# articulatory/articulatory

Measured on AMD Instinct MI355X. Metric: audio samples/sec (16 kHz) EMA->wav HiFi-CAR, batch 64, higher is better.
Workload: dtype fp32; 1 GPU; configs[2]: HiFi-CAR (e2w_hifigan_car.yaml generator) 13-dim pitch+EMA -> 16 kHz, batch 64/GPU, 10 s clips, 80 sequential chunks of 25 frames; batch_per_gpu=64, frames=2000, chunk_frames=25, weights=synthetic seed 1234 (articulatory_amd.utils.synth), parallelism=utterance-sharded x1, arithmetic=exact fp32 products (v_mfma_f32_32x32x2_f32), fp32 accumulate, gather=none

## Files before the change

__graft_entry__.py:

```python

import os
import subprocess
import sys

REPO = os.path.dirname(os.path.abspath(__file__))
if REPO not in sys.path:
    sys.path.insert(0, REPO)


def build() -> None:
    csrc = os.path.join(REPO, "articulatory_amd", "csrc")
    subprocess.run(["make", "-C", csrc, f"-j{max(1, min(11, os.cpu_count() or 1))}"], check=True)
    import articulatory_amd
    from articulatory_amd import _native

    lib = _native.load_library()
    for sym in _native.SYMBOLS:
        getattr(lib, sym)
    print("built", _native.LIB_PATH, lib.hificar_version().decode())


def smoke() -> None:
    import numpy as np
    import torch

    from articulatory_amd.models import HiFiGANGenerator
    from articulatory_amd.utils.synth import synth_features, synth_state_dict
# ... 47 lines not shown
```

articulatory_amd/csrc/hificar.hip:

```cpp
#include "hificar_kernels.hip.h"
#include "hificar_launch.h"
#include "hificar_backward.hip.h"
#include "hificar_disc_kernels.hip.h"

#include "../../include/hificar.h"

#include <algorithm>
#include <queue>
#include <cmath>
#include <cstdarg>
#include <cstdio>
#include <cstring>
#include <functional>
#include <map>
#include <string>
#include <vector>

using namespace hificar;

static thread_local char g_err[1024] = "";

static int fail(int code, const char* fmt, ...) {
    va_list ap;
    va_start(ap, fmt);
// ... 44 lines not shown
struct hificar_handle {
    hificar_config cfg;
    int arch = 0;
    std::vector<GBlockLayers> gb;
    int c_last = 0;
    bool finalized = false;
    int precision = HIFICAR_PREC_F32;
    bool profile_detail = false;
    bool use_pair = true;
    bool use_lpt = true;
    double mi1_penalty = 1.05;
    int pick_throughput = 0;
    bool xcd_order = true;
    bool pair_small = true;
    int ksplit = 1;
    int cf = 0;
    int cin_pad = 0;
    int hop = 1;
    int num_cus = 256;
    std::map<std::string, std::vector<int64_t>> expected;
    std::map<std::string, HostTensor> tensors;
    ConvLayer input_conv;
    std::vector<ConvLayer> ups;
    std::vector<ConvLayer> convs1;
    std::vector<ConvLayer> convs2;
    float* d_out_w = nullptr;
    float out_bias = 0.f;
    float* d_out_bias = nullptr;
    void* train = nullptr;
    void (*train_free)(hificar_handle*) = nullptr;
// ... 62 lines not shown
    hipStream_t prof_stream = nullptr;
};

static FILE* g_launch_log = nullptr;
static void read_env_switches(hificar_handle* h) {
    if (const char* e = getenv("HIFICAR_PROFILE_DETAIL")) h->profile_detail = atoi(e) != 0;
    if (const char* e = getenv("HIFICAR_LAUNCH_LOG")) {
        if (!g_launch_log && *e) g_launch_log = fopen(e, "a");
        if (g_launch_log) h->profile_detail = true;
    }
    if (const char* e = getenv("HIFICAR_KSPLIT")) h->ksplit = atoi(e);
    if (const char* e = getenv("HIFICAR_PAIR")) h->use_pair = atoi(e) != 0;
    if (const char* e = getenv("HIFICAR_PAIR_SMALL")) h->pair_small = atoi(e) != 0;
    if (const char* e = getenv("HIFICAR_AR_DUAL_MIN")) h->ar_dual_min = atoi(e);
    if (const char* e = getenv("HIFICAR_AR_DUAL_MAX")) h->ar_dual_max = atoi(e);
}

struct ProfScope {
    hificar_handle* h;
    hipStream_t s;
    hipEvent_t e0 = nullptr, e1 = nullptr;
    std::string name;
    double flops, bytes;
    ProfScope(hificar_handle* h_, hipStream_t s_, const std::string& n, double f, double b) : h(h_), s(s_), name(n), flops(f), bytes(b) {
        if (g_launch_log) {
            fprintf(g_launch_log, "%s\t%.0f\t%.0f\n", n.c_str(), f, b);
            fflush(g_launch_log);
        }
        if (!h->profiling) return;
        (void)hipEventCreate(&e0);
// ... 376 lines not shown
    if (!L.transposed && L.cin_pad == L.cin && (L.cin == 32 || L.cin == 64) && L.cout == L.cin) {
        if ((rc = pack_w16(h, L, W, L.cin_pad, &L.d_w16c)) != HIFICAR_OK) return rc;
        if ((rc = pack_w32(h, L, W, L.cin_pad, &L.d_w32c)) != HIFICAR_OK) return rc;
    }
    return HIFICAR_OK;
}

hipError_t hificar::conv_launch(const ConvShape& s, const void* params, dim3 grid, size_t lds_bytes, hipStream_t stream) {
    bool handled = false;
    hipError_t e = hipSuccess;
#define HIFICAR_TRY_SET(n)                                                      \
    if (!handled) e = conv_inst_launch_##n(s, params, grid, lds_bytes, stream, &handled); \
    if (handled) return e;
    HIFICAR_TRY_SET(0) HIFICAR_TRY_SET(1) HIFICAR_TRY_SET(2) HIFICAR_TRY_SET(3) HIFICAR_TRY_SET(4)
    HIFICAR_TRY_SET(5) HIFICAR_TRY_SET(6) HIFICAR_TRY_SET(7) HIFICAR_TRY_SET(8) HIFICAR_TRY_SET(9)
#undef HIFICAR_TRY_SET
    return hipErrorInvalidValue;
}

hipError_t hificar::conv_set_lds_attributes() {
    hipError_t e = hipSuccess;
#define HIFICAR_ATTR_SET(n) \
    if (e == hipSuccess) e = conv_inst_attrs_##n();
    HIFICAR_ATTR_SET(0) HIFICAR_ATTR_SET(1) HIFICAR_ATTR_SET(2) HIFICAR_ATTR_SET(3) HIFICAR_ATTR_SET(4)
    HIFICAR_ATTR_SET(5) HIFICAR_ATTR_SET(6) HIFICAR_ATTR_SET(7) HIFICAR_ATTR_SET(8) HIFICAR_ATTR_SET(9)
#undef HIFICAR_ATTR_SET
    return e;
}

static int engine_setup(hificar_handle* h) {
    {
        void* z = nullptr;
        HIP_TRY(hipMalloc(&z, 256));
        h->allocs.push_back(z);
        HIP_TRY(hipMemset(z, 0, 256));
        h->d_zeros = static_cast<char*>(z);
    }
    HIP_TRY(conv_set_lds_attributes());
    if (h->arenas.empty()) {
        int rca = arena_add(h, 0);
// ... 347 lines not shown
    float mask_slope = 0.f;
    long long x_seq_bytes = 0;
    int x_row_bytes = 0;
    int x_rows = 0;
    int x_up = 0;
    float x_slope = -1.f;
    const float* x_more[3] = {nullptr, nullptr, nullptr};
    int x_n = 1;
};

struct ConvRep {
    int n = 1;
    long long zs_x = 0, zs_w = 0, zs_y = 0, zs_b = 0;
};

static int launch_conv(hificar_handle* h, const ConvLayer* const* layers, int nbr, int nseq, int rows, const ConvIO* io,
                              float slope_out, const Ragged& rg, hipStream_t stream, const ConvRep& zr = ConvRep()) {
    const ConvLayer& L0 = *layers[0];
    const bool f32 = h->precision == HIFICAR_PREC_F32;
    int halo_all = 0;
    for (int b = 0; b < nbr; ++b) halo_all = std::max(halo_all, layers[b]->off_max - layers[b]->off_min);
    TileCfg tc = {1, 4, 1, 1, 1};
    double best = 1e300;
    int best_ti = 11;
    const int nsteps_min = [&] {
        int m = 1 << 30;
        for (int b = 0; b < nbr; ++b) m = std::min(m, layers[b]->ntaps * (L0.chunk16 / 16));
        return m;
    }();
    std::string pick_key;
    pick_key.reserve(160);
    pick_key += f32 ? 'f' : 'c';
    pick_key += h->train ? 't' : 'i';
    if (h->shared_chip) pick_key += 's';
    for (int b = 0; b < nbr; ++b) {
        pick_key += '|';
        pick_key += layers[b]->name;
    }
    pick_key += '|' + std::to_string(nseq) + 'x' + std::to_string(rows) + 'z' + std::to_string(zr.n);
    const auto cached_pick = h->tile_picks.find(pick_key);
    if (cached_pick != h->tile_picks.end()) tc = kTileCfgs[cached_pick->second];
    else
    for (int ti = 0; ti < kNumTileCfgs; ++ti) {
        const TileCfg& t = kTileCfgs[ti];
        const int TM = t.WM * t.MI * 32;
        const int chunk = L0.chunk16, RB = chunk * 4;
        if (t.NB == 2 && (f32 || L0.chunk16 == 16)) continue;
        const size_t obuf = (f32 && t.KS == 1) ? 0 : out_buf_bytes(t);
        if (2 * round_up_sz((size_t)(TM + halo_all) * RB, 1024) + obuf > 160 * 1024) continue;
        if (t.NB == 2) {
            bool ok = L0.n_blocks32 >= 2;
            for (int b = 0; b < nbr; ++b) ok = ok && (layers[b]->n_phase == 1 || layers[b]->nb32_per_phase % 2 == 0);
            if (!ok) continue;
        }
        if (t.KS == 4 && (h->ksplit == 0 || nsteps_min < 2)) continue;
        if (t.KS == 1 && h->ksplit == 2 && nsteps_min >= 2) continue;
        const long long tiles_per_branch = (long long)nseq * ((rows + TM - 1) / TM) * ((L0.n_blocks32 + t.WN * t.NB - 1) / (t.WN * t.NB));
        const long long total = tiles_per_branch * nbr * zr.n;
        const int G = (int)std::min<long long>(total, h->num_cus);
        const int nchunks = L0.cin_pad / chunk;
        double total_cost = 0.0, heaviest = 0.0, lightest = 1e300, cb[3] = {0.0, 0.0, 0.0};
        for (int b = 0; b < nbr; ++b) {
            const double slab = f32 ? 8 * 64.0 : 3 * 32 / 0.75;
            double c = (double)layers[b]->ntaps * (L0.cin_pad / 16) * slab * t.MI * t.NB + 2500.0 + 400.0 * nchunks;
            if (t.KS == 4) {
                const int steps = layers[b]->ntaps * (chunk / 16);
                c = (double)((steps + 3) / 4) * nchunks * slab * t.MI + 4000.0 + 600.0 * nchunks;
            }
            total_cost += c * tiles_per_branch * zr.n;
            heaviest = std::max(heaviest, c);
            lightest = std::min(lightest, c);
            cb[b] = c;
        }
        double worst = std::max(heaviest, total_cost / G);
        if (h->use_lpt && !h->shared_chip && total > G && total <= 4096) {
            std::sort(cb, cb + nbr, [](double x, double y) { return x > y; });
            std::priority_queue<double, std::vector<double>, std::greater<double>> load;
            for (int w = 0; w < G; ++w) load.push(0.0);
            worst = 0.0;
            for (int b = 0; b < nbr; ++b)
                for (long long i = 0; i < tiles_per_branch * zr.n; ++i) {
                    const double v = load.top() + cb[b];
                    load.pop();
                    load.push(v);
                    worst = std::max(worst, v);
                }
        } else if (total % G != 0) {
            worst = std::max(worst, total_cost / G + 0.5 * lightest);
        }
        if (h->pick_throughput > 0 && total >= h->pick_throughput) worst = total_cost / h->num_cus;
        if (t.NB == 2) worst *= f32 ? (t.MI == 4 ? 0.95 : t.MI == 2 ? 0.975 : 1.02) : (t.MI == 2 ? 0.93 : 1.10);
        else if (t.MI < 4) worst *= f32 ? (t.MI == 2 ? 1.02 : h->mi1_penalty) : (t.MI == 2 ? 1.10 : 1.25);
        if (t.KS == 4) worst *= 1.05;
        if (worst < best * 0.98) {
            best = worst;
            tc = t;
            best_ti = ti;
        }
    }
    if (cached_pick == h->tile_picks.end()) {
        if (h->tile_picks.size() > 20000) h->tile_picks.clear();
        h->tile_picks.emplace(pick_key, best_ti);
    }
    const int TM = tc.WM * tc.MI * 32;
    const int chunk_sel = L0.chunk16, RB = chunk_sel * 4;
    const int nc16 = chunk_sel / 16;
    MultiConvParams mp;
    memset(&mp, 0, sizeof(mp));
    double flops = 0.0, bytes = 0.0;
    for (int b = 0; b < nbr; ++b) {
        const ConvLayer& Lb = *layers[b];
        if (Lb.n_blocks32 != L0.n_blocks32 || Lb.chunk16 != L0.chunk16 || Lb.cin_pad != L0.cin_pad)
            return fail(HIFICAR_E_INVALID, "internal: branch shape mismatch");
        fill_params(mp.p[b], Lb, rows, TM, io[b].res, io[b].y, rg);
        mp.p[b].xs = io[b].xs;
        mp.p[b].ys = io[b].ys;
        if (io[b].x_slope >= 0.f) {
            if (!f32) return fail(HIFICAR_E_INVALID, "internal: pre-activation input rows of %s outside the exact-fp32 layer-by-layer launches", Lb.name.c_str());
// ... 33 lines not shown
    mp.buf_bytes = (int)buf_bytes;
    mp.trace = nullptr;
    mp.zrep = zr.n;
    mp.zs_x = zr.zs_x;
    mp.zs_w = zr.zs_w;
    mp.zs_y = zr.zs_y;
    mp.zs_b = zr.zs_b;
    dim3 grid((unsigned)std::min(mp.total_tiles, h->num_cus), 1, 1);
    {
        double wbytes = 0.0;
        for (int b = 0; b < nbr; ++b) wbytes += 4.0 * layers[b]->cin_pad * layers[b]->cout_total * layers[b]->ntaps * zr.n;
        const double abytes = 4.0 * nseq * rows * L0.cin_pad * nbr * zr.n;
        mp.xcd_order = (h->xcd_order && mp.total_tiles <= h->num_cus && mp.total_tiles >= 16 && wbytes > 2.0 * abytes) ? 1 : 0;
    }
    mp.stage_cached = mp.ngroups > 2 ? 1 : 0;
    if (mp.total_tiles <= h->num_cus && nbr == 1 && zr.n == 1 && mp.ngroups >= 2 && mp.nseq_tiles >= 8 && !h->shared_chip) {
        const double wbytes1 = 4.0 * L0.cin_pad * L0.cout_total * L0.ntaps;
        if (wbytes1 > 6.0e6) {
            const int R = mp.nseq_tiles, Gc = mp.ngroups;
            int bpr = 1, bpg = 8;
            double bcost = 1e300;
            for (int pr = 1; pr <= 8; pr *= 2) {
                const int pg = 8 / pr;
                if (pr > R || pg > Gc) continue;
                const double c = (double)((R + pr - 1) / pr) + (double)((Gc + pg - 1) / pg);
                if (c < bcost) bcost = c, bpr = pr, bpg = pg;
            }
            std::vector<std::vector<int>> per_xcd(8);
            size_t maxblock = 0;
            for (int x = 0; x < 8; ++x) {
// ... 19 lines not shown
    if (!mp.sched_start && h->use_lpt && mp.total_tiles > (int)grid.x) {
        std::vector<double> costs((size_t)mp.total_tiles);
        const int tpb = mp.ngroups * mp.nseq_tiles;
        std::string key = f32 ? "f" : "c";
        for (int b = 0; b < nbr; ++b) {
            key += "|" + layers[b]->name;
            for (int i = 0; i < tpb * zr.n; ++i) costs[(size_t)b * tpb * zr.n + i] = layers[b]->ntaps + 1.0;
        }
        if (zr.n > 1) key += "z" + std::to_string(zr.n);
        key += "|" + std::to_string(nseq) + "x" + std::to_string((rows + TM - 1) / TM) + "t" + std::to_string(TM) + "w" + std::to_string(tc.WN) +
               "k" + std::to_string(tc.KS) + (tc.NB == 2 ? "b" : "");
        int rc2 = get_schedule(h, key, costs, (int)grid.x, stream, &mp.sched_start, &mp.sched_tiles);
        if (rc2 != HIFICAR_OK) return rc2;
    }
    char kname[96];
    if (dout) snprintf(kname, sizeof(kname), "conv_f32do_kernel<%d,%d,%d,%d>", tc.MI, tc.WM, tc.WN, nc16);
    else if (tc.KS == 4) snprintf(kname, sizeof(kname), "%s<%d,%d>", f32 ? "conv_sk_f32_kernel" : "conv_sk_bf16x3_kernel", tc.MI, nc16);
    else if (tc.NB == 2) snprintf(kname, sizeof(kname), "conv_bf16x3nb_kernel<%d,%d,%d,%d>", tc.MI, tc.WM, tc.WN, nc16);
    else snprintf(kname, sizeof(kname), "conv_bf16x3_kernel<%d,%d,%d,%d>", tc.MI, tc.WM, tc.WN, nc16);
    if (h->profile_detail) {
        const size_t n = strlen(kname);
        snprintf(kname + n, sizeof(kname) - n, "|%s x%d", L0.name.c_str(), nbr);
    }
    ProfScope prof(h, stream, kname, flops, bytes);
    const ConvShape shape = {dout ? kConvF32do : tc.KS == 4 ? (f32 ? kConvSkF32 : kConvSkBf16x3) : tc.NB == 2 ? kConvBf16x3nb : kConvBf16x3,
                             tc.MI, tc.WM, tc.WN, nc16};
    const hipError_t e = conv_launch(shape, &mp, grid, lds, stream);
    if (e != hipSuccess) return fail(HIFICAR_E_HIP, "conv launch (%s, %s) failed: %s", L0.name.c_str(), kname, hipGetErrorString(e));
    return HIFICAR_OK;
}

struct PairIOB {
    const float* xf;
    const char* xs;
    const float* res;
    float* y;
    char* ys;
};

static bool pair_small_tiles(const hificar_handle* h, int C, int k2, int nseq, int rows) {
    if (!h->pair_small || h->ksplit == 0 || C != 32 || h->precision != HIFICAR_PREC_F32 || nseq <= 0 || (long long)nseq * rows < 8000) return false;
    const int tmo = 4 * 4 * 32 - (k2 - 1);
// ... 249 lines not shown
            h->tap_scratch = static_cast<float*>(p);
            h->tap_scratch_elems = need;
        }
        if (cfg.use_ar && (rc = emit_tap(h, "ar_feats", ws.xin, f32 ? h->cin_pad : -h->cin_pad, h->cf, cfg.ar_output, B, 1, f32 ? 0 : 1, stream, T)) != HIFICAR_OK)
            return rc;
    }
    const size_t tap_se = tapping ? stage_elems(h, B, T) : 0;
    const int nbk = cfg.n_blocks;
    int order[kMaxBlk];
    for (int j = 0; j < kMaxBlk; ++j) order[j] = j;
    std::sort(order, order + nbk, [&](int a, int b) { return cfg.resblock_kernel_sizes[a] > cfg.resblock_kernel_sizes[b]; });
    int max_d = 0;
    for (int j = 0; j < nbk; ++j) max_d = std::max(max_d, cfg.n_dilations[j]);
    int rows_of_launch = 0;
    const bool add_convs = cfg.use_additional_convs != 0;
    auto conv_n = [&](const ConvLayer* const* lay, int n, const ConvIO* io) -> int {
        for (int q0 = 0; q0 < n; q0 += 3) {
            const int r = launch_conv(h, lay + q0, std::min(3, n - q0), B, rows_of_launch, io + q0, cfg.lrelu_slope, rg, stream);
            if (r != HIFICAR_OK) return r;
        }
        return HIFICAR_OK;
    };

    const float* fin[kMaxBlk] = {ws.x[0], ws.x[1], ws.x[2], ws.x[3]};
    {
        char* xin_s = tp ? reinterpret_cast<char*>(tp->xin) : reinterpret_cast<char*>(ws.xin);
        char* h0_s = tp ? tp->h0_s : reinterpret_cast<char*>(ws.h0);
        char* xt_s[kMaxBlk] = {reinterpret_cast<char*>(ws.xt[0]), reinterpret_cast<char*>(ws.xt[1]), reinterpret_cast<char*>(ws.xt[2]),
                               reinterpret_cast<char*>(ws.xt[3])};
        {
            const ConvLayer* lay[1] = {&h->input_conv};
            float* y_tap = tap_wanted(h, "input_conv") ? h->tap_scratch + kMaxBlk * tap_se : nullptr;
            const ConvIO io[1] = {{xin_s, nullptr, y_tap, h0_s}};
            if ((rc = launch_conv(h, lay, 1, B, T, io, cfg.lrelu_slope, rg, stream)) != HIFICAR_OK) return rc;
            if (y_tap && (rc = emit_tap(h, "input_conv", y_tap, stage_pad(cfg, 0), 0, cfg.channels, B, T, 0, stream)) != HIFICAR_OK) return rc;
        }
        for (int i = 0; i < cfg.n_stages; ++i) {
            const char* up_in = h0_s;
            const bool fold_mrf = i > 0 && f32 && !tp;
            if (i > 0 && !fold_mrf) {
                MrfSplitParams mq;
                memset(&mq, 0, sizeof(mq));
                mq.x0 = fin[0];
                mq.x1 = nbk > 1 ? fin[1] : nullptr;
                mq.x2 = nbk > 2 ? fin[2] : nullptr;
                mq.x3 = nbk > 3 ? fin[3] : nullptr;
                mq.out = fin[0] == ws.xt[0] ? ws.x_s[0] : xt_s[0];
                if (tp) mq.out = tp->upin_s[i];
                mq.nin = nbk;
                mq.C = stage_pad(cfg, i);
                mq.rows = (long long)B * rows;
                mq.slope = cfg.lrelu_slope;
                mq.f32 = f32 ? 1 : 0;
                const long long units = mq.rows * (mq.C / 8);
// ... 2 lines not shown
                    ProfScope prof(h, stream, "mrf_split_kernel", 0.0, 4.0 * mq.rows * mq.C * (nbk + 1));
                    hipLaunchKernelGGL(mrf_split_kernel, dim3(blocks), dim3(256), 0, stream, mq);
                }
                HIP_TRY(hipGetLastError());
                up_in = mq.out;
            }
            bool all_pairs = !tap_convs1 && !tp && add_convs;
            for (int j = 0; j < nbk && all_pairs; ++j)
                for (int d = 0; d < cfg.n_dilations[j]; ++d) {
                    const int ci = conv_index(h, i, j, d);
                    all_pairs = all_pairs && pair_eligible(h, h->convs1[ci], h->convs2[ci], B, rows * cfg.upsample_scales[i]);
                }
            {
                const ConvLayer* lay[1] = {&h->ups[i]};
                ConvIO io[1] = {{up_in, nullptr, ws.u, all_pairs ? nullptr : (tp ? tp->u_s[i] : ws.u_s)}};
                if (fold_mrf) {
                    io[0].xs = reinterpret_cast<const char*>(fin[0]);
                    io[0].x_slope = cfg.lrelu_slope;
                    io[0].x_n = nbk;
                    for (int j = 1; j < nbk; ++j) io[0].x_more[j - 1] = fin[j];
                }
                if ((rc = launch_conv(h, lay, 1, B, rows, io, cfg.lrelu_slope, rg, stream)) != HIFICAR_OK) return rc;
            }
            rows *= cfg.upsample_scales[i];
            const int Cs = stage_channels(cfg, i + 1), Cp = stage_pad(cfg, i + 1);
            if (tapping && (rc = emit_tap(h, "upsamples." + std::to_string(i), ws.u, Cp, 0, Cs, B, rows, 0, stream)) != HIFICAR_OK) return rc;
            auto tap_block = [&](int j, int d, const float* xcur) -> int {
                if (!tapping) return HIFICAR_OK;
                const std::string base = "blocks." + std::to_string(i * nbk + j);
                int r = emit_tap(h, base + ".x." + std::to_string(d), xcur, Cp, 0, Cs, B, rows, 0, stream);
                if (r == HIFICAR_OK && d + 1 == cfg.n_dilations[j]) r = emit_tap(h, base, xcur, Cp, 0, Cs, B, rows, 0, stream);
// ... 19 lines not shown
                    }
                    for (int q0 = 0; q0 < n; q0 += 3)
                        if ((rc = launch_pair(h, l1 + q0, l2 + q0, std::min(3, n - q0), B, rows, iop + q0, cfg.lrelu_slope, rg, stream)) != HIFICAR_OK) return rc;
                    for (int j = 0; j < nbk; ++j)
                        if (d < cfg.n_dilations[j] && (rc = tap_block(j, d, cur_f[j])) != HIFICAR_OK) return rc;
                }
                for (int j = 0; j < nbk; ++j) fin[j] = cur_f[j];
                continue;
            }
            float* xres[kMaxBlk] = {ws.x[0], ws.x[1], ws.x[2], ws.x[3]};
            if (tp && i + 1 == cfg.n_stages)
                for (int j = 0; j < nbk; ++j) xres[j] = tp->fin[j];
            for (int j = 0; j < nbk; ++j) fin[j] = xres[j];
            const char* u_act = tp ? tp->u_s[i] : ws.u_s;
            const char* cur_s[kMaxBlk] = {u_act, u_act, u_act, u_act};
            for (int d = 0; d < max_d; ++d) {
                const ConvLayer* l1[kMaxBlk];
                const ConvLayer* l2[kMaxBlk];
                ConvIO io1[kMaxBlk], io2[kMaxBlk];
                PairIOB iop[kMaxBlk];
                int jn[kMaxBlk];
                char* pair_out[kMaxBlk];
                char* lbl_out[kMaxBlk];
                int n = 0;
                bool fuse = add_convs;
                for (int oj = 0; oj < nbk; ++oj) {
                    const int j = order[oj];
                    if (d >= cfg.n_dilations[j]) continue;
                    const int ci = conv_index(h, i, j, d);
                    l1[n] = &h->convs1[ci];
// ... 6 lines not shown
                    if (tp) {
                        mid = tp->xt_s[i][j][d];
                        lbl_out[n] = tp->x_s[i][j][d];
                    }
                    io1[n] = {cur_s[j], nullptr, tap_convs1 ? h->tap_scratch + (size_t)n * tap_se : nullptr, mid};
                    io2[n] = {mid, d == 0 ? ws.u : xres[j], xres[j], last ? nullptr : lbl_out[n]};
                    if (!add_convs) {
                        char* nxt = tp ? tp->x_s[i][j][d] : pair_out[n];
                        io1[n] = {cur_s[j], d == 0 ? ws.u : xres[j], xres[j], last ? nullptr : nxt};
                        lbl_out[n] = nxt;
                    }
                    iop[n] = {nullptr, cur_s[j], d == 0 ? ws.u : xres[j], xres[j], last ? nullptr : pair_out[n]};
                    jn[n] = j;
                    ++n;
                }
                if (fuse) {
                    for (int q0 = 0; q0 < n; q0 += 3)
                        if ((rc = launch_pair(h, l1 + q0, l2 + q0, std::min(3, n - q0), B, rows, iop + q0, cfg.lrelu_slope, rg, stream)) != HIFICAR_OK) return rc;
                } else if (!add_convs) {
                    rows_of_launch = rows;
                    if ((rc = conv_n(l1, n, io1)) != HIFICAR_OK) return rc;
                } else {
                    rows_of_launch = rows;
                    if ((rc = conv_n(l1, n, io1)) != HIFICAR_OK) return rc;
                    if (tap_convs1)
                        for (int q = 0; q < n; ++q)
                            if ((rc = emit_tap(h, "blocks." + std::to_string(i * nbk + jn[q]) + ".convs1." + std::to_string(d), io1[q].y, Cp, 0, Cs,
                                               B, rows, 0, stream)) != HIFICAR_OK)
                                return rc;
                    if ((rc = conv_n(l2, n, io2)) != HIFICAR_OK) return rc;
                }
                for (int q = 0; q < n; ++q)
                    if ((rc = tap_block(jn[q], d, xres[jn[q]])) != HIFICAR_OK) return rc;
                for (int q = 0; q < n; ++q) cur_s[jn[q]] = fuse ? pair_out[q] : lbl_out[q];
            }
        }
    }
    if (cfg.use_ph_loss && cond.ph_out) {
        PhHeadParams pq;
        memset(&pq, 0, sizeof(pq));
        pq.x0 = fin[0];
        pq.x1 = nbk > 1 ? fin[1] : nullptr;
        pq.x2 = nbk > 2 ? fin[2] : nullptr;
        pq.x3 = nbk > 3 ? fin[3] : nullptr;
        pq.nin = nbk;
        pq.w = h->d_phfc_w;
// ... 287 lines not shown
```

articulatory_amd/csrc/hificar_conv.hip.h:

```cpp
#pragma once
#include <hip/hip_runtime.h>
#include <stdint.h>
#include <type_traits>

namespace hificar {

typedef float f32x2 __attribute__((ext_vector_type(2)));
typedef float f32x4 __attribute__((ext_vector_type(4)));
typedef unsigned u32x4_t __attribute__((ext_vector_type(4)));
typedef float f32x16 __attribute__((ext_vector_type(16)));
typedef __bf16 bf16x4 __attribute__((ext_vector_type(4)));
typedef __bf16 bf16x8 __attribute__((ext_vector_type(8)));

constexpr int kMaxPhase = 8;
constexpr int kMaxTaps = 16;

struct ConvParams {
    const bf16x8* w16;
    const float* bias;
    const float* res;
    const float* mask_src;
    float mask_slope;
    float* y;
    const float* xf;
// ... 51 lines not shown
    ConvParams p[3];
    int n_branches;
    int nseq_tiles;
    int ngroups;
    int total_tiles;
    int buf_bytes;
    const int* sched_start;
    const int* sched_tiles;
    int zrep;
    long long zs_x, zs_w, zs_y, zs_b;
    unsigned long long* trace;
    int xcd_order;
    int stage_cached;
};


#ifdef HIFICAR_TRACE
__device__ unsigned long long g_trace_realtime[2][1024];
__device__ unsigned long long g_trace_rt_slots[4][64];
#define HIFICAR_STAMP(slot)                                                                            \
    do {                                                                                               \
        if (mp.trace && lane == 0 && (wave == 0 || wave == kFirstLoader) && (slot) < 64)               \
            mp.trace[((size_t)blockIdx.x * 2 + (wave ? 1 : 0)) * 64 + (slot)] = __builtin_amdgcn_s_memtime(); \
        if (mp.trace && lane == 0 && wave == 0 && ((slot) == 0 || (slot) == 63) && blockIdx.x < 1024)  \
            g_trace_realtime[(slot) == 63][blockIdx.x] = __builtin_amdgcn_s_memrealtime();             \
        if (mp.trace && lane == 0 && wave == 0 && (slot) < 64 && blockIdx.x < 4)                       \
            g_trace_rt_slots[blockIdx.x][(slot)] = __builtin_amdgcn_s_memrealtime();                   \
    } while (0)
#else
#define HIFICAR_STAMP(slot) do { } while (0)
// ... 9 lines not shown
        constexpr int lo = NMEM * I / NMFMA, hi = NMEM * (I + 1) / NMFMA;
        constexpr int ds = (hi < NDS ? hi : NDS) - (lo < NDS ? lo : NDS);
        constexpr int vm = (hi - lo) - ds;
        __builtin_amdgcn_sched_group_barrier(0x008, 1, 0);
        if constexpr (ds > 0) __builtin_amdgcn_sched_group_barrier(0x100, ds, 0);
        if constexpr (vm > 0) __builtin_amdgcn_sched_group_barrier(0x020, vm, 0);
        pin_slab_slot<I + 1, NDS, NVMEM, NMFMA>();
    }
}
template <int NDS, int NVMEM, int NMFMA>
__device__ __forceinline__ void pin_slab_step() {
    pin_slab_slot<0, NDS, NVMEM, NMFMA>();
}
__device__ __forceinline__ void lds_barrier() { asm volatile("s_waitcnt lgkmcnt(0)\n\ts_barrier" ::: "memory"); }

template <int MI, int WM, int WN, int NC16, bool F32, int KS = 1, int NB = 1, bool DOUT = false>
__device__ __forceinline__ void conv_ws_body(const MultiConvParams& mp) {
    static_assert(!DOUT || (F32 && KS == 1 && NB == 1), "direct output: exact fp32, dense form, one channel block per wave");
    static_assert(NB == 1 || (NB == 2 && KS == 1), "one or two channel blocks per MFMA wave");
    static_assert(KS == 1 || (KS == 4 && WM == 1 && WN == 1), "split-K: four waves share one 32-channel block");
    static_assert(KS == 4 || WM * WN == 4 || WM * WN == 8, "4 or 8 MFMA waves per workgroup");
    constexpr int NW = KS == 4 ? 4 : WM * WN;
    constexpr bool kPrimeOnce = DOUT;
    constexpr bool kRowMajorAcc = DOUT;
    constexpr int NTHR = (NW + 4) * 64;
    constexpr int kFirstLoader = NW;
    (void)kFirstLoader;
    static_assert(NC16 == 1 || NC16 == 2 || NC16 == 4, "chunk of 16, 32 or 64 channels");
    constexpr int TM = WM * MI * 32;
    constexpr int CH = NC16 * 16;
    constexpr int RB = CH * 4;
    constexpr int SPR = CH / 4;
    constexpr int LOG_SPR = NC16 == 4 ? 4 : NC16 == 2 ? 3 : 2;
// ... 30 lines not shown
        const unsigned tps = (unsigned)mp.p[0].tiles_per_seq;
        const unsigned seq = m / tps;
        T.seq = (int)seq;
        T.t0 = (int)((m - seq * tps) * (unsigned)TM);
        return T;
    };

    constexpr int TN = WN * NB * 32;
    constexpr int OP = TN + 4;
    int sched_lo = 0, sched_hi = 0;
    if (mp.sched_start) scalar_load_2i32(mp.sched_start + blockIdx.x, sched_lo, sched_hi);
    const int my_rounds = mp.sched_start ? sched_hi - sched_lo
                                         : (mp.total_tiles - (int)blockIdx.x + (int)gridDim.x - 1) / (int)gridDim.x;
    auto tile_of = [&](int it) {
        int i = it;
        if ((blockIdx.x & 1) && my_rounds >= 3 && it >= my_rounds - 2) i = it == my_rounds - 1 ? my_rounds - 2 : my_rounds - 1;
        if (mp.sched_start) return scalar_load_i32(mp.sched_tiles + sched_lo + i);
        if (mp.xcd_order) {
            const int x = (int)blockIdx.x & 7, l = (int)blockIdx.x >> 3;
            const int base = mp.total_tiles >> 3, rem = mp.total_tiles & 7;
            return x * base + min(x, rem) + l;
        }
        return (int)blockIdx.x + (my_rounds - 1 - i) * (int)gridDim.x;
    };
    auto nxt = [&](int i) {
        if (is_ragged(mp.p[0]))
            while (i < my_rounds) {
                const Tile T = decode(tile_of(i));
                if (T.t0 < seq_rows(mp.p[T.b], T.seq)) break;
                ++i;
            }
// ... 410 lines not shown
                    for (int m0 = 0; m0 < MI; m0 += G2) {
                        float rs[G2][16], mk[G2][16];
                        if constexpr (kRes || kMask) {
#pragma unroll
                            for (int mm = 0; mm < G2; ++mm)
#pragma unroll
                                for (int r = 0; r < 16; ++r) fetch1(m0 + mm, r, rs[mm], mk[mm]);
                        }
#pragma unroll
                        for (int mm = 0; mm < G2; ++mm)
#pragma unroll
                            for (int r = 0; r < 16; ++r) finish(m0 + mm, r, rs[mm], mk[mm]);
                    }
                }
            };
            constexpr std::true_type Y{};
            constexpr std::false_type N{};
            if (has_mask) {
                pass(Y, Y, Y, Y);
                return;
            }
            if (has_res) {
                if (has_y && has_ys) pass(Y, N, Y, Y);
                else if (has_y) pass(Y, N, Y, N);
                else pass(Y, N, N, Y);
            } else {
                if (has_y && has_ys) pass(N, N, Y, Y);
                else if (has_y) pass(N, N, Y, N);
                else pass(N, N, N, Y);
            }
// ... 232 lines not shown
    }
    lds_barrier();
    HIFICAR_STAMP(62);
    if constexpr (!DOUT) {
        if (last >= 0) write_out(decode(tile_of(last)), tid, NTHR);
    }
    HIFICAR_STAMP(63);
}

template <int MI, int WM, int WN, int NC16>
__global__ __launch_bounds__((WM * WN + 4) * 64) void conv_f32do_kernel(const MultiConvParams mp) {
    conv_ws_body<MI, WM, WN, NC16, true, 1, 1, true>(mp);
}

template <int MI, int WM, int WN, int NC16>
__global__ __launch_bounds__((WM * WN + 4) * 64) void conv_bf16x3_kernel(const MultiConvParams mp) {
    conv_ws_body<MI, WM, WN, NC16, false>(mp);
}

template <int MI, int WM, int WN, int NC16>
__global__ __launch_bounds__((WM * WN + 4) * 64) void conv_bf16x3nb_kernel(const MultiConvParams mp) {
    conv_ws_body<MI, WM, WN, NC16, false, 1, 2>(mp);
}

template <int MI, int NC16>
__global__ __launch_bounds__(512) void conv_sk_bf16x3_kernel(const MultiConvParams mp) {
    conv_ws_body<MI, 1, 1, NC16, false, 4>(mp);
}

template <int MI, int NC16>
// ... 476 lines not shown
```

articulatory_amd/csrc/hificar_conv_inst.hip:

```cpp
#include "hificar_conv.hip.h"
#include "hificar_launch.h"

#ifndef HIFICAR_INST_SET
#error "compile with -DHIFICAR_INST_SET=0..9"
#endif

namespace hificar {

#define HIFICAR_TILES9(X, nc) X(4, 1, 4, nc) X(4, 2, 2, nc) X(4, 4, 1, nc) X(2, 1, 4, nc) X(2, 2, 2, nc) X(2, 4, 1, nc) X(1, 1, 4, nc) X(1, 2, 2, nc) X(1, 4, 1, nc)

#if HIFICAR_INST_SET == 0
#define FAMILY kConvF32do
#define KERNEL conv_f32do_kernel
#define PARAMS MultiConvParams
#define SHAPES(X) HIFICAR_TILES9(X, 1)
#elif HIFICAR_INST_SET == 1
#define FAMILY kConvF32do
#define KERNEL conv_f32do_kernel
#define PARAMS MultiConvParams
#define SHAPES(X) HIFICAR_TILES9(X, 2)
#elif HIFICAR_INST_SET == 2
#define FAMILY kConvF32do
#define KERNEL conv_f32do_kernel
#define PARAMS MultiConvParams
// ... 17 lines not shown
#define FAMILY kConvBf16x3nb
#define KERNEL conv_bf16x3nb_kernel
#define PARAMS MultiConvParams
#define SHAPES(X) X(2, 2, 2, 2) X(2, 4, 1, 2) X(2, 1, 4, 2) X(2, 2, 2, 4) X(2, 4, 1, 4) X(2, 1, 4, 4)
#elif HIFICAR_INST_SET == 7 || HIFICAR_INST_SET == 8
#if HIFICAR_INST_SET == 7
#define FAMILY kConvSkF32
#define KERNEL_PTR(mi, wm, wn, nc) (conv_sk_f32_kernel<mi, nc>)
#else
#define FAMILY kConvSkBf16x3
#define KERNEL_PTR(mi, wm, wn, nc) (conv_sk_bf16x3_kernel<mi, nc>)
#endif
#define THREADS(wm, wn) 512
#define PARAMS MultiConvParams
#define SHAPES(X) X(1, 1, 1, 1) X(2, 1, 1, 1) X(4, 1, 1, 1) X(1, 1, 1, 2) X(2, 1, 1, 2) X(4, 1, 1, 2) X(1, 1, 1, 4) X(2, 1, 1, 4) X(4, 1, 1, 4)
#elif HIFICAR_INST_SET == 9
#define PARAMS PairParams
#define THREADS(wm, wn) 512
#else
#error "HIFICAR_INST_SET out of range"
#endif

#ifndef KERNEL_PTR
#define KERNEL_PTR(mi, wm, wn, nc) (KERNEL<mi, wm, wn, nc>)
#endif
#ifndef THREADS
#define THREADS(wm, wn) ((wm * wn + 4) * 64)
#endif

#define HIFICAR_CAT_(a, b) a##b
// ... 67 lines not shown
```

articulatory_amd/csrc/hificar_launch.h:

```cpp
#pragma once
#include <hip/hip_runtime.h>

namespace hificar {

struct MultiConvParams;
struct PairParams;

enum ConvFamily {
    kConvF32do = 0,
    kConvBf16x3 = 1,
    kConvBf16x3nb = 2,
    kConvSkF32 = 3,
    kConvSkBf16x3 = 4,
    kPairF32 = 5,
    kPairBf16x3 = 6,
};

struct ConvShape {
    int family, mi, wm, wn, nc16;
};

hipError_t conv_launch(const ConvShape& s, const void* params, dim3 grid, size_t lds_bytes, hipStream_t stream);
hipError_t conv_set_lds_attributes();

#define HIFICAR_N_INST_SETS 10
#define HIFICAR_DECL_SET(n)                                                                                                              \
    hipError_t conv_inst_launch_##n(const ConvShape& s, const void* params, dim3 grid, size_t lds, hipStream_t stream, bool* handled); \
    hipError_t conv_inst_attrs_##n();
HIFICAR_DECL_SET(0) HIFICAR_DECL_SET(1) HIFICAR_DECL_SET(2) HIFICAR_DECL_SET(3) HIFICAR_DECL_SET(4)
HIFICAR_DECL_SET(5) HIFICAR_DECL_SET(6) HIFICAR_DECL_SET(7) HIFICAR_DECL_SET(8) HIFICAR_DECL_SET(9)
#undef HIFICAR_DECL_SET

}
```

Measured before the change: 39.60 million samples/s.

## Fuse MRF branch mean and leaky-ReLU into last resblock conv epilogue

```diff
diff --git a/__graft_entry__.py b/__graft_entry__.py
--- a/__graft_entry__.py
+++ b/__graft_entry__.py
@@ -10,7 +10,7 @@
 
 def build() -> None:
     csrc = os.path.join(REPO, "articulatory_amd", "csrc")
-    subprocess.run(["make", "-C", csrc, f"-j{max(1, min(11, os.cpu_count() or 1))}"], check=True)
+    subprocess.run(["make", "-C", csrc, f"-j{max(1, min(13, os.cpu_count() or 1))}"], check=True)
     import articulatory_amd
     from articulatory_amd import _native
 
diff --git a/articulatory_amd/csrc/hificar.hip b/articulatory_amd/csrc/hificar.hip
--- a/articulatory_amd/csrc/hificar.hip
+++ b/articulatory_amd/csrc/hificar.hip
@@ -82,6 +82,7 @@
     bool xcd_order = true;
     bool pair_small = true;
     int ksplit = 1;
+    bool mrf_fold_producer = true;
     int cf = 0;
     int cin_pad = 0;
     int hop = 1;
@@ -174,6 +175,7 @@
     if (const char* e = getenv("HIFICAR_PAIR_SMALL")) h->pair_small = atoi(e) != 0;
     if (const char* e = getenv("HIFICAR_AR_DUAL_MIN")) h->ar_dual_min = atoi(e);
     if (const char* e = getenv("HIFICAR_AR_DUAL_MAX")) h->ar_dual_max = atoi(e);
+    if (const char* e = getenv("HIFICAR_MRF_FOLD")) h->mrf_fold_producer = atoi(e) != 0;
 }
 
 struct ProfScope {
@@ -580,6 +582,7 @@
     if (handled) return e;
     HIFICAR_TRY_SET(0) HIFICAR_TRY_SET(1) HIFICAR_TRY_SET(2) HIFICAR_TRY_SET(3) HIFICAR_TRY_SET(4)
     HIFICAR_TRY_SET(5) HIFICAR_TRY_SET(6) HIFICAR_TRY_SET(7) HIFICAR_TRY_SET(8) HIFICAR_TRY_SET(9)
+    HIFICAR_TRY_SET(10) HIFICAR_TRY_SET(11)
 #undef HIFICAR_TRY_SET
     return hipErrorInvalidValue;
 }
@@ -590,6 +593,7 @@
     if (e == hipSuccess) e = conv_inst_attrs_##n();
     HIFICAR_ATTR_SET(0) HIFICAR_ATTR_SET(1) HIFICAR_ATTR_SET(2) HIFICAR_ATTR_SET(3) HIFICAR_ATTR_SET(4)
     HIFICAR_ATTR_SET(5) HIFICAR_ATTR_SET(6) HIFICAR_ATTR_SET(7) HIFICAR_ATTR_SET(8) HIFICAR_ATTR_SET(9)
+    HIFICAR_ATTR_SET(10) HIFICAR_ATTR_SET(11)
 #undef HIFICAR_ATTR_SET
     return e;
 }
@@ -967,15 +971,29 @@
     long long zs_x = 0, zs_w = 0, zs_y = 0, zs_b = 0;
 };
 
+struct MrfOut {
+    float* out;
+    float slope;
+    int rank[3];
+    bool done = false;
+};
+
+static std::vector<std::vector<int>> mrf_unit_lists(int nunits, int nbr, const int* rank, int G) {
+    int branch_of[3] = {0, 0, 0};
+    for (int b = 0; b < nbr; ++b) branch_of[rank[b]] = b;
+    std::vector<std::vector<int>> lists((size_t)std::min(nunits, G));
+    for (int u = 0; u < nunits; ++u)
+        for (int k = 0; k < nbr; ++k) lists[(size_t)(u % (int)lists.size())].push_back(branch_of[k] * nunits + u);
+    return lists;
+}
+
 static int launch_conv(hificar_handle* h, const ConvLayer* const* layers, int nbr, int nseq, int rows, const ConvIO* io,
-                              float slope_out, const Ragged& rg, hipStream_t stream, const ConvRep& zr = ConvRep()) {
+                              float slope_out, const Ragged& rg, hipStream_t stream, const ConvRep& zr = ConvRep(), MrfOut* mo = nullptr) {
     const ConvLayer& L0 = *layers[0];
     const bool f32 = h->precision == HIFICAR_PREC_F32;
     int halo_all = 0;
     for (int b = 0; b < nbr; ++b) halo_all = std::max(halo_all, layers[b]->off_max - layers[b]->off_min);
     TileCfg tc = {1, 4, 1, 1, 1};
-    double best = 1e300;
-    int best_ti = 11;
     const int nsteps_min = [&] {
         int m = 1 << 30;
         for (int b = 0; b < nbr; ++b) m = std::min(m, layers[b]->ntaps * (L0.chunk16 / 16));
@@ -991,11 +1009,12 @@
         pick_key += layers[b]->name;
     }
     pick_key += '|' + std::to_string(nseq) + 'x' + std::to_string(rows) + 'z' + std::to_string(zr.n);
-    const auto cached_pick = h->tile_picks.find(pick_key);
-    if (cached_pick != h->tile_picks.end()) tc = kTileCfgs[cached_pick->second];
-    else
+    auto evaluate = [&](bool units, double& best) -> int {
+    best = 1e300;
+    int best_ti = 11;
     for (int ti = 0; ti < kNumTileCfgs; ++ti) {
         const TileCfg& t = kTileCfgs[ti];
+        if (units && t.KS != 1) continue;
         const int TM = t.WM * t.MI * 32;
         const int chunk = L0.chunk16, RB = chunk * 4;
         if (t.NB == 2 && (f32 || L0.chunk16 == 16)) continue;
@@ -1010,7 +1029,7 @@
         if (t.KS == 1 && h->ksplit == 2 && nsteps_min >= 2) continue;
         const long long tiles_per_branch = (long long)nseq * ((rows + TM - 1) / TM) * ((L0.n_blocks32 + t.WN * t.NB - 1) / (t.WN * t.NB));
         const long long total = tiles_per_branch * nbr * zr.n;
-        const int G = (int)std::min<long long>(total, h->num_cus);
+        const int G = (int)std::min<long long>(units ? tiles_per_branch : total, h->num_cus);
         const int nchunks = L0.cin_pad / chunk;
         double total_cost = 0.0, heaviest = 0.0, lightest = 1e300, cb[3] = {0.0, 0.0, 0.0};
         for (int b = 0; b < nbr; ++b) {
@@ -1026,7 +1045,11 @@
             cb[b] = c;
         }
         double worst = std::max(heaviest, total_cost / G);
-        if (h->use_lpt && !h->shared_chip && total > G && total <= 4096) {
+        if (units) {
+            double unit_cost = 0.0;
+            for (int b = 0; b < nbr; ++b) unit_cost += cb[b];
+            worst = (double)((tiles_per_branch + G - 1) / G) * unit_cost;
+        } else if (h->use_lpt && !h->shared_chip && total > G && total <= 4096) {
             std::sort(cb, cb + nbr, [](double x, double y) { return x > y; });
             std::priority_queue<double, std::vector<double>, std::greater<double>> load;
             for (int w = 0; w < G; ++w) load.push(0.0);
@@ -1047,14 +1070,32 @@
         if (t.KS == 4) worst *= 1.05;
         if (worst < best * 0.98) {
             best = worst;
-            tc = t;
             best_ti = ti;
         }
     }
-    if (cached_pick == h->tile_picks.end()) {
+    return best_ti;
+    };
+    auto cached = [&](const std::string& key, auto compute) -> int {
+        const auto it = h->tile_picks.find(key);
+        if (it != h->tile_picks.end()) return it->second;
         if (h->tile_picks.size() > 20000) h->tile_picks.clear();
-        h->tile_picks.emplace(pick_key, best_ti);
-    }
+        const int v = compute();
+        h->tile_picks.emplace(key, v);
+        return v;
+    };
+    int pick_ti = cached(pick_key, [&] { double c; return evaluate(false, c); });
+    bool mean_units = mo && f32 && kTileCfgs[pick_ti].KS == 1 && zr.n == 1 && (nbr == 2 || nbr == 3) && L0.chunk16 >= 32;
+    if (mean_units) {
+        const int m = cached(pick_key + 'm', [&] {
+            double c_plain, c_units;
+            evaluate(false, c_plain);
+            const int ti = evaluate(true, c_units);
+            return c_units <= 1.05 * c_plain ? ti : -1;
+        });
+        if (m >= 0) pick_ti = m;
+        else mean_units = false;
+    }
+    tc = kTileCfgs[pick_ti];
     const int TM = tc.WM * tc.MI * 32;
     const int chunk_sel = L0.chunk16, RB = chunk_sel * 4;
     const int nc16 = chunk_sel / 16;
@@ -1118,6 +1159,29 @@
         mp.xcd_order = (h->xcd_order && mp.total_tiles <= h->num_cus && mp.total_tiles >= 16 && wbytes > 2.0 * abytes) ? 1 : 0;
     }
     mp.stage_cached = mp.ngroups > 2 ? 1 : 0;
+    MeanConvParams mq;
+    const bool mean_out = mean_units && dout;
+    if (mean_out) {
+        memset(&mq.mean, 0, sizeof(mq.mean));
+        for (int b = 0; b < nbr; ++b) {
+            if (!io[b].res || !io[b].y || mo->rank[b] < 0 || mo->rank[b] >= nbr) return fail(HIFICAR_E_INVALID, "internal: MRF mean-out launch %s", L0.name.c_str());
+            if (mo->rank[b] == nbr - 1) mq.mean.b = b;
+            else mq.mean.y[mo->rank[b]] = io[b].y;
+        }
+        mq.mean.n = nbr;
+        mq.mean.out = mo->out;
+        mq.mean.slope = mo->slope;
+        const int nunits = mp.ngroups * mp.nseq_tiles;
+        const auto lists = mrf_unit_lists(nunits, nbr, mo->rank, h->num_cus);
+        std::string key = "f|mrf";
+        for (int b = 0; b < nbr; ++b) key += "|" + layers[b]->name + ":" + std::to_string(mo->rank[b]);
+        key += "|" + std::to_string(nseq) + "x" + std::to_string(mp.nseq_tiles / nseq) + "t" + std::to_string(TM) + "w" + std::to_string(tc.WN);
+        grid = dim3((unsigned)lists.size(), 1, 1);
+        mp.xcd_order = 0;
+        int rc2 = put_schedule(h, key, lists, mp.total_tiles, stream, &mp.sched_start, &mp.sched_tiles);
+        if (rc2 != HIFICAR_OK) return rc2;
+        bytes += 4.0 * nseq * rows * L0.cout_total * (nbr - 1);
+    }
     if (mp.total_tiles <= h->num_cus && nbr == 1 && zr.n == 1 && mp.ngroups >= 2 && mp.nseq_tiles >= 8 && !h->shared_chip) {
         const double wbytes1 = 4.0 * L0.cin_pad * L0.cout_total * L0.ntaps;
         if (wbytes1 > 6.0e6) {
@@ -1167,7 +1231,8 @@
         if (rc2 != HIFICAR_OK) return rc2;
     }
     char kname[96];
-    if (dout) snprintf(kname, sizeof(kname), "conv_f32do_kernel<%d,%d,%d,%d>", tc.MI, tc.WM, tc.WN, nc16);
+    if (mean_out) snprintf(kname, sizeof(kname), "conv_f32dom_kernel<%d,%d,%d,%d>", tc.MI, tc.WM, tc.WN, nc16);
+    else if (dout) snprintf(kname, sizeof(kname), "conv_f32do_kernel<%d,%d,%d,%d>", tc.MI, tc.WM, tc.WN, nc16);
     else if (tc.KS == 4) snprintf(kname, sizeof(kname), "%s<%d,%d>", f32 ? "conv_sk_f32_kernel" : "conv_sk_bf16x3_kernel", tc.MI, nc16);
     else if (tc.NB == 2) snprintf(kname, sizeof(kname), "conv_bf16x3nb_kernel<%d,%d,%d,%d>", tc.MI, tc.WM, tc.WN, nc16);
     else snprintf(kname, sizeof(kname), "conv_bf16x3_kernel<%d,%d,%d,%d>", tc.MI, tc.WM, tc.WN, nc16);
@@ -1176,9 +1241,11 @@
         snprintf(kname + n, sizeof(kname) - n, "|%s x%d", L0.name.c_str(), nbr);
     }
     ProfScope prof(h, stream, kname, flops, bytes);
-    const ConvShape shape = {dout ? kConvF32do : tc.KS == 4 ? (f32 ? kConvSkF32 : kConvSkBf16x3) : tc.NB == 2 ? kConvBf16x3nb : kConvBf16x3,
+    const ConvShape shape = {mean_out ? kConvF32dom : dout ? kConvF32do : tc.KS == 4 ? (f32 ? kConvSkF32 : kConvSkBf16x3) : tc.NB == 2 ? kConvBf16x3nb : kConvBf16x3,
                              tc.MI, tc.WM, tc.WN, nc16};
-    const hipError_t e = conv_launch(shape, &mp, grid, lds, stream);
+    if (mean_out) mq.mp = mp;
+    const hipError_t e = mean_out ? conv_launch(shape, &mq, grid, lds, stream) : conv_launch(shape, &mp, grid, lds, stream);
+    if (mo) mo->done = mean_out && e == hipSuccess;
     if (e != hipSuccess) return fail(HIFICAR_E_HIP, "conv launch (%s, %s) failed: %s", L0.name.c_str(), kname, hipGetErrorString(e));
     return HIFICAR_OK;
 }
@@ -1458,9 +1525,9 @@
     for (int j = 0; j < nbk; ++j) max_d = std::max(max_d, cfg.n_dilations[j]);
     int rows_of_launch = 0;
     const bool add_convs = cfg.use_additional_convs != 0;
-    auto conv_n = [&](const ConvLayer* const* lay, int n, const ConvIO* io) -> int {
+    auto conv_n = [&](const ConvLayer* const* lay, int n, const ConvIO* io, MrfOut* mo = nullptr) -> int {
         for (int q0 = 0; q0 < n; q0 += 3) {
-            const int r = launch_conv(h, lay + q0, std::min(3, n - q0), B, rows_of_launch, io + q0, cfg.lrelu_slope, rg, stream);
+            const int r = launch_conv(h, lay + q0, std::min(3, n - q0), B, rows_of_launch, io + q0, cfg.lrelu_slope, rg, stream, ConvRep(), n <= 3 ? mo : nullptr);
             if (r != HIFICAR_OK) return r;
         }
         return HIFICAR_OK;
@@ -1479,9 +1546,12 @@
             if ((rc = launch_conv(h, lay, 1, B, T, io, cfg.lrelu_slope, rg, stream)) != HIFICAR_OK) return rc;
             if (y_tap && (rc = emit_tap(h, "input_conv", y_tap, stage_pad(cfg, 0), 0, cfg.channels, B, T, 0, stream)) != HIFICAR_OK) return rc;
         }
+        const char* mrf_act = nullptr;
         for (int i = 0; i < cfg.n_stages; ++i) {
             const char* up_in = h0_s;
             const bool fold_mrf = i > 0 && f32 && !tp;
+            const char* mrf_in = mrf_act;
+            mrf_act = nullptr;
             if (i > 0 && !fold_mrf) {
                 MrfSplitParams mq;
                 memset(&mq, 0, sizeof(mq));
@@ -1514,7 +1584,9 @@
             {
                 const ConvLayer* lay[1] = {&h->ups[i]};
                 ConvIO io[1] = {{up_in, nullptr, ws.u, all_pairs ? nullptr : (tp ? tp->u_s[i] : ws.u_s)}};
-                if (fold_mrf) {
+                if (fold_mrf && mrf_in) {
+                    io[0].xs = mrf_in;
+                } else if (fold_mrf) {
                     io[0].xs = reinterpret_cast<const char*>(fin[0]);
                     io[0].x_slope = cfg.lrelu_slope;
                     io[0].x_n = nbk;
@@ -1564,6 +1636,8 @@
             for (int j = 0; j < nbk; ++j) fin[j] = xres[j];
             const char* u_act = tp ? tp->u_s[i] : ws.u_s;
             const char* cur_s[kMaxBlk] = {u_act, u_act, u_act, u_act};
+            bool mrf_producer = h->mrf_fold_producer && f32 && !tp && !tapping && i + 1 < cfg.n_stages && (nbk == 2 || nbk == 3);
+            for (int j = 0; j < nbk; ++j) mrf_producer = mrf_producer && cfg.n_dilations[j] == max_d;
             for (int d = 0; d < max_d; ++d) {
                 const ConvLayer* l1[kMaxBlk];
                 const ConvLayer* l2[kMaxBlk];
@@ -1600,12 +1674,20 @@
                     jn[n] = j;
                     ++n;
                 }
+                MrfOut mrf;
+                MrfOut* mo = nullptr;
+                if (mrf_producer && d + 1 == max_d && !fuse) {
+                    mrf.out = reinterpret_cast<float*>(add_convs ? lbl_out[0] : pair_out[0]);
+                    mrf.slope = cfg.lrelu_slope;
+                    for (int q = 0; q < n; ++q) mrf.rank[q] = jn[q];
+                    mo = &mrf;
+                }
                 if (fuse) {
                     for (int q0 = 0; q0 < n; q0 += 3)
                         if ((rc = launch_pair(h, l1 + q0, l2 + q0, std::min(3, n - q0), B, rows, iop + q0, cfg.lrelu_slope, rg, stream)) != HIFICAR_OK) return rc;
                 } else if (!add_convs) {
                     rows_of_launch = rows;
-                    if ((rc = conv_n(l1, n, io1)) != HIFICAR_OK) return rc;
+                    if ((rc = conv_n(l1, n, io1, mo)) != HIFICAR_OK) return rc;
                 } else {
                     rows_of_launch = rows;
                     if ((rc = conv_n(l1, n, io1)) != HIFICAR_OK) return rc;
@@ -1614,8 +1696,9 @@
                             if ((rc = emit_tap(h, "blocks." + std::to_string(i * nbk + jn[q]) + ".convs1." + std::to_string(d), io1[q].y, Cp, 0, Cs,
                                                B, rows, 0, stream)) != HIFICAR_OK)
                                 return rc;
-                    if ((rc = conv_n(l2, n, io2)) != HIFICAR_OK) return rc;
+                    if ((rc = conv_n(l2, n, io2, mo)) != HIFICAR_OK) return rc;
                 }
+                if (mrf.done) mrf_act = reinterpret_cast<const char*>(mrf.out);
                 for (int q = 0; q < n; ++q)
                     if ((rc = tap_block(jn[q], d, xres[jn[q]])) != HIFICAR_OK) return rc;
                 for (int q = 0; q < n; ++q) cur_s[jn[q]] = fuse ? pair_out[q] : lbl_out[q];
diff --git a/articulatory_amd/csrc/hificar_conv.hip.h b/articulatory_amd/csrc/hificar_conv.hip.h
--- a/articulatory_amd/csrc/hificar_conv.hip.h
+++ b/articulatory_amd/csrc/hificar_conv.hip.h
@@ -89,6 +89,18 @@
     int stage_cached;
 };
 
+struct MrfMeanParams {
+    int b;
+    int n;
+    const float* y[2];
+    float* out;
+    float slope;
+};
+struct MeanConvParams {
+    MultiConvParams mp;
+    MrfMeanParams mean;
+};
+
 
 #ifdef HIFICAR_TRACE
 __device__ unsigned long long g_trace_realtime[2][1024];
@@ -128,9 +140,10 @@
 }
 __device__ __forceinline__ void lds_barrier() { asm volatile("s_waitcnt lgkmcnt(0)\n\ts_barrier" ::: "memory"); }
 
-template <int MI, int WM, int WN, int NC16, bool F32, int KS = 1, int NB = 1, bool DOUT = false>
-__device__ __forceinline__ void conv_ws_body(const MultiConvParams& mp) {
+template <int MI, int WM, int WN, int NC16, bool F32, int KS = 1, int NB = 1, bool DOUT = false, bool MEAN = false>
+__device__ __forceinline__ void conv_ws_body(const MultiConvParams& mp, const MrfMeanParams& mq = MrfMeanParams()) {
     static_assert(!DOUT || (F32 && KS == 1 && NB == 1), "direct output: exact fp32, dense form, one channel block per wave");
+    static_assert(!MEAN || DOUT, "the MRF mean is written by the direct-output epilogue");
     static_assert(NB == 1 || (NB == 2 && KS == 1), "one or two channel blocks per MFMA wave");
     static_assert(KS == 1 || (KS == 4 && WM == 1 && WN == 1), "split-K: four waves share one 32-channel block");
     static_assert(KS == 4 || WM * WN == 4 || WM * WN == 8, "4 or 8 MFMA waves per workgroup");
@@ -191,7 +204,7 @@
                                          : (mp.total_tiles - (int)blockIdx.x + (int)gridDim.x - 1) / (int)gridDim.x;
     auto tile_of = [&](int it) {
         int i = it;
-        if ((blockIdx.x & 1) && my_rounds >= 3 && it >= my_rounds - 2) i = it == my_rounds - 1 ? my_rounds - 2 : my_rounds - 1;
+        if (!MEAN && (blockIdx.x & 1) && my_rounds >= 3 && it >= my_rounds - 2) i = it == my_rounds - 1 ? my_rounds - 2 : my_rounds - 1;
         if (mp.sched_start) return scalar_load_i32(mp.sched_tiles + sched_lo + i);
         if (mp.xcd_order) {
             const int x = (int)blockIdx.x & 7, l = (int)blockIdx.x >> 3;
@@ -632,6 +645,34 @@
                     }
                 }
             };
+            if constexpr (MEAN) {
+                if (T.b == mq.b) {
+                    asm volatile("s_waitcnt vmcnt(0)" ::: "memory");
+                    const int n = mq.n;
+                    const unsigned long long b_y0 = uni64((unsigned long long)(mq.y[0] + first));
+                    const unsigned long long b_y1 = uni64((unsigned long long)(n == 3 ? mq.y[1] + first : nullptr));
+                    const unsigned long long b_m = uni64((unsigned long long)(mq.out + first));
+                    const float slope_m = mq.slope;
+#pragma unroll
+                    for (int mi = 0; mi < MI; ++mi) {
+                        float rs[16], v0[16], v1[16];
+#pragma unroll
+                        for (int r = 0; r < 16; ++r) {
+                            rs[r] = __builtin_bit_cast(float, __builtin_amdgcn_raw_buffer_load_b32(rsrc_of(b_res, has_res, mi), off16[r], 0, 0));
+                            v0[r] = __builtin_bit_cast(float, __builtin_amdgcn_raw_buffer_load_b32(rsrc_of(b_y0, true, mi), off16[r], 0, 0));
+                            v1[r] = __builtin_bit_cast(float, __builtin_amdgcn_raw_buffer_load_b32(rsrc_of(b_y1, n == 3, mi), off16[r], 0, 0));
+                        }
+#pragma unroll
+                        for (int r = 0; r < 16; ++r) {
+                            float o = acc[0][mi][r] + bias_l;
+                            o += rs[r];
+                            const float m = n == 3 ? ((v0[r] + v1[r]) + o) / 3.0f : (v0[r] + o) / 2.0f;
+                            __builtin_amdgcn_raw_buffer_store_b32(__builtin_bit_cast(unsigned, fmaxf(m, m * slope_m)), rsrc_of(b_m, true, mi), off16[r], 0, kAux);
+                        }
+                    }
+                    return;
+                }
+            }
             constexpr std::true_type Y{};
             constexpr std::false_type N{};
             if (has_mask) {
@@ -894,6 +935,11 @@
 }
 
 template <int MI, int WM, int WN, int NC16>
+__global__ __launch_bounds__((WM * WN + 4) * 64) void conv_f32dom_kernel(const MeanConvParams q) {
+    conv_ws_body<MI, WM, WN, NC16, true, 1, 1, true, true>(q.mp, q.mean);
+}
+
+template <int MI, int WM, int WN, int NC16>
 __global__ __launch_bounds__((WM * WN + 4) * 64) void conv_bf16x3_kernel(const MultiConvParams mp) {
     conv_ws_body<MI, WM, WN, NC16, false>(mp);
 }
diff --git a/articulatory_amd/csrc/hificar_conv_inst.hip b/articulatory_amd/csrc/hificar_conv_inst.hip
--- a/articulatory_amd/csrc/hificar_conv_inst.hip
+++ b/articulatory_amd/csrc/hificar_conv_inst.hip
@@ -2,7 +2,7 @@
 #include "hificar_launch.h"
 
 #ifndef HIFICAR_INST_SET
-#error "compile with -DHIFICAR_INST_SET=0..9"
+#error "compile with -DHIFICAR_INST_SET=0..11"
 #endif
 
 namespace hificar {
@@ -55,6 +55,16 @@
 #define THREADS(wm, wn) 512
 #define PARAMS MultiConvParams
 #define SHAPES(X) X(1, 1, 1, 1) X(2, 1, 1, 1) X(4, 1, 1, 1) X(1, 1, 1, 2) X(2, 1, 1, 2) X(4, 1, 1, 2) X(1, 1, 1, 4) X(2, 1, 1, 4) X(4, 1, 1, 4)
+#elif HIFICAR_INST_SET == 10
+#define FAMILY kConvF32dom
+#define KERNEL conv_f32dom_kernel
+#define PARAMS MeanConvParams
+#define SHAPES(X) HIFICAR_TILES9(X, 2)
+#elif HIFICAR_INST_SET == 11
+#define FAMILY kConvF32dom
+#define KERNEL conv_f32dom_kernel
+#define PARAMS MeanConvParams
+#define SHAPES(X) HIFICAR_TILES9(X, 4)
 #elif HIFICAR_INST_SET == 9
 #define PARAMS PairParams
 #define THREADS(wm, wn) 512
diff --git a/articulatory_amd/csrc/hificar_launch.h b/articulatory_amd/csrc/hificar_launch.h
--- a/articulatory_amd/csrc/hificar_launch.h
+++ b/articulatory_amd/csrc/hificar_launch.h
@@ -5,6 +5,7 @@
 
 struct MultiConvParams;
 struct PairParams;
+struct MeanConvParams;
 
 enum ConvFamily {
     kConvF32do = 0,
@@ -14,6 +15,7 @@
     kConvSkBf16x3 = 4,
     kPairF32 = 5,
     kPairBf16x3 = 6,
+    kConvF32dom = 7,
 };
 
 struct ConvShape {
@@ -23,12 +25,13 @@
 hipError_t conv_launch(const ConvShape& s, const void* params, dim3 grid, size_t lds_bytes, hipStream_t stream);
 hipError_t conv_set_lds_attributes();
 
-#define HIFICAR_N_INST_SETS 10
+#define HIFICAR_N_INST_SETS 12
 #define HIFICAR_DECL_SET(n)                                                                                                              \
     hipError_t conv_inst_launch_##n(const ConvShape& s, const void* params, dim3 grid, size_t lds, hipStream_t stream, bool* handled); \
     hipError_t conv_inst_attrs_##n();
 HIFICAR_DECL_SET(0) HIFICAR_DECL_SET(1) HIFICAR_DECL_SET(2) HIFICAR_DECL_SET(3) HIFICAR_DECL_SET(4)
 HIFICAR_DECL_SET(5) HIFICAR_DECL_SET(6) HIFICAR_DECL_SET(7) HIFICAR_DECL_SET(8) HIFICAR_DECL_SET(9)
+HIFICAR_DECL_SET(10) HIFICAR_DECL_SET(11)
 #undef HIFICAR_DECL_SET
 
 }
```

Result: no change. 39.67 million samples/s, median of 6 (+0.2%).
